# h3poteto/aws-global-accelerator-controller

Hardware: NVIDIA H100
Metric: objects reconciled/sec at 10^6 Service+Ingress; change-set bit-exact vs Go ref (higher is better)
Workload: dtype u8/u32 (bytes and indices)

## Files before the change

### aws-global-accelerator-controller_b200/csrc/gar_common.h

```cpp
#pragma once

#include <stdint.h>
#include <stddef.h>

#include "../../include/garecon.h"

#if defined(__CUDACC__)
#define GAR_HD __host__ __device__ __forceinline__
#define GAR_D __device__ __forceinline__
#else
#define GAR_HD inline
#define GAR_D inline
#endif

#if defined(__CUDA_ARCH__)
#define GAR_ANY(p) __any_sync(0xffffffffu, (p))
#else
bool gar_host_vote(bool p);
#define GAR_ANY(p) gar_host_vote((p))
#endif

typedef uint8_t u8;
typedef uint16_t u16;
typedef uint32_t u32;
// ... 206 lines not shown
#else
  return *p;
#endif
}

GAR_HD Cursor idx_open(const HashIdx &ix, u64 h) {
  u32 b = hash_bucket(h, ix.mask);
  Cursor c;
  c.pos = ix.begin[b];
  c.end = ix.begin[b + 1];
  c.tag = hash_tag(h);
  return c;
}
GAR_HD bool idx_next(const HashIdx &ix, Cursor &c, IdxEntry *out) {
  while (c.pos < c.end) {
    IdxEntry e = load_entry(ix.ent + c.pos++);
    if (e.tag == c.tag) {
      *out = e;
      return true;
    }
  }
  return false;
}
```

### aws-global-accelerator-controller_b200/csrc/gar_pipeline.h

```cpp
#pragma once

#include <stdio.h>
#include <stdlib.h>

#include <initializer_list>

#include "gar_rows.h"

#if defined(__CUDA_ARCH__)
#define GAR_ATOMIC_ADD(p, v) atomicAdd((p), (v))
#else
#define GAR_ATOMIC_ADD(p, v) (*(p) += (v))
#endif


enum Slot {
  S_DERIVED, S_OFLAGS, S_OKEY_HASH, S_STAGE_GA, S_STAGE_R53, S_ANN_R53, S_ANN_NAME, S_ANN_TAGS, S_ANN_LISTEN, S_DPORT_BEGIN, S_DPORTS,
  S_TOK_CODE, S_TOK_NAME, S_TOK_REGION,
  S_ACC_FLAGS, S_ACC_OWNER_KEY, S_ACC_OWNER, S_ACC_THOST, S_ACC_MANAGED, S_ACC_OWNER_HASH, S_ACC_THOST_HASH, S_REC_NAME_HASH, S_VAL_KEY_HASH,
  S_REC_ZONE, S_VAL_REC, S_VAL_CLS, S_VAL_KEY, S_VAL_ORPHAN, S_VAL_LINK, S_ACC_DIGEST,
  S_R53_MODE, S_R53_ACC, S_R53_ACC_DNS, S_PAIR_BEGIN, S_PAIR_OBJ, S_PAIR_HN, S_PAIR_CODE, S_PAIR_ZONE, S_PAIR_REC,
  S_IX_LB, S_IX_OWNER = S_IX_LB + 3, S_IX_THOST = S_IX_OWNER + 3, S_IX_ZONE = S_IX_THOST + 3, S_IX_VAL = S_IX_ZONE + 3,
  S_IX_ALIAS = S_IX_VAL + 3, S_IX_OBJ = S_IX_ALIAS + 3, S_IX_OVN = S_IX_OBJ + 3,
  S_SORT_KEYS = S_IX_OVN + 3, S_SORT_VALS, S_SORT_KEYS_ALT, S_SORT_VALS_ALT, S_SORT_TAGS,
  S_COUNTS, S_STATUS_GA, S_STATUS_R53, S_OPS, S_ERRFLAG, S_IX_EG, S_IX_EG_ENT, S_IX_EG_PAD,
  S_VAL_OBJ, S_ACC_OBJ, S_OBJ_CANON, S_OWN_BEGIN, S_OWN_FILL, S_OWN_ENT, S_OWN_MULTI,
  S_IXA_BEGIN, S_IXA_FILL, S_IXA_ENT, S_IXA_MULTI, S_OVN_FILL, S_OVN_MULTI, S_LB_HASH, S_REC_FLAGS,
  S_NSLOTS
};


struct FClassify {
  DevTables T;
  Work W;
  u32 *derived_public;
  u8 *oflags;
  u32 *errflag;
  GAR_HD void operator()(u32 i) const {
    classify_object(T, W, i);
    W.obj_canon[i] = i;
    u32 dv = W.derived[i];
    if (dv & OBJ_KEY_BAD) GAR_ATOMIC_ADD(errflag, 1u);
    derived_public[i] = dv & 0xFFu;
  }
};
struct FTokenise {
  DevTables T;
  Work W;
  static constexpr int kStageCols = 1;
  static constexpr u32 kStageBytes = 24 * 1024;
// ... 438 lines not shown
  GAR_HD void operator()(u32 k) const { dst[k] = k < 5 ? src[idx[k]] : *extra; }
};
#define GAR_RETRY_WITH_RADIX 1000
#define GAR_REFUSE_EMPTY_CACHE 1001
struct FGatherHeader {
  const u32 *ndports;
  u32 *flags;
  GAR_HD void operator()(u32) const { flags[FW_NDPORTS] = *ndports; }
};
struct FValueJoins {
  DevTables T;
  Work W;
  GAR_HD void operator()(u32 v) const { value_joins(T, W, v); }
};
struct FResolveValue {
  DevTables T;
  Work W;
  GAR_HD void operator()(u32 v) const { resolve_value(T, W, v); }
};
struct FResolveAccel {
  DevTables T;
  Work W;
  GAR_HD void operator()(u32 a) const { resolve_accel(T, W, a); }
};
GAR_HD IdxEntry own_entry(const DevTables &T, const Work &W, u32 x) {
  IdxEntry e;
  e.tag = e.a0 = e.a1 = 0;
  e.s0 = e.s1 = 0;
  if (x < T.a.n_accels) {
    e.row = x;
    return e;
  }
  const u32 v = x - T.a.n_accels, rec = W.val_rec[v];
  const ValLink l = W.val_link[v];
  e.tag = l.alias_row;
  e.row = v;
  e.a0 = rec;
  e.a1 = W.rec_zone[rec] | ((W.rec_flags[rec] & 1) ? VALNAME_HAS_BACKSLASH : 0u);
  e.s0 = l.alias_dns;
  e.s1 = T.a.rec_name[rec];
  return e;
}
GAR_HD u32 own_segment(const DevTables &T, const Work &W, u32 x) {
  const u32 nacc = T.a.n_accels;
  const u32 o = x < nacc ? W.acc_obj[x] : W.val_obj[x - nacc];
  return o == GAR_NONE ? 2 * T.o.n_objects : 2 * o + (x < nacc ? 0u : 1u);
// ... 316 lines not shown
  }

  bool prepared = false;
  u64 n_dports = 0;
  u32 *errflag = nullptr;

  u32 acc_guest_from = 0xFFFFFFFFu;
  u32 sharded = 0;
  bool orphan_sweep = true;
  bool allow_empty_cache = false;

  void alloc_obj_work() {
    const u32 n = T.o.n_objects, nlbi = T.o.n_lbi;
    W.derived = (u32 *)be.ensure(S_DERIVED, 4 * (size_t)(n + 1));
    W.okey_hash = (u64 *)be.ensure(S_OKEY_HASH, 8 * (size_t)(n + 1));
    W.ann_r53 = (gar_str *)be.ensure(S_ANN_R53, 8 * (size_t)(n + 1));
    W.ann_name = (gar_str *)be.ensure(S_ANN_NAME, 8 * (size_t)(n + 1));
    W.ann_tags = (gar_str *)be.ensure(S_ANN_TAGS, 8 * (size_t)(n + 1));
    W.ann_listen = (gar_str *)be.ensure(S_ANN_LISTEN, 8 * (size_t)(n + 1));
    W.dport_begin = (u32 *)be.out_dport_begin(n);
    W.tok_code = (u8 *)be.out_tok_code(nlbi);
    W.tok_name = (gar_str *)be.out_tok_name(nlbi);
    W.tok_region = (gar_str *)be.out_tok_region(nlbi);
    W.r53_mode = (u8 *)be.ensure(S_R53_MODE, (size_t)n + 1);
    W.r53_acc = (u32 *)be.ensure(S_R53_ACC, 4 * (size_t)(n + 1));
    W.r53_acc_dns = (gar_str *)be.ensure(S_R53_ACC_DNS, 8 * (size_t)(n + 1));
    W.obj_canon = (u32 *)be.ensure(S_OBJ_CANON, 4 * (size_t)(n + 1));
  }
  CanonHook canon_hook(u32 b0, u32 b1) const { return CanonHook{W.obj_canon, T.o.slab, b0, b1}; }
  void alloc_work() {
    const u32 nacc = T.a.n_accels, nrec = T.a.n_records, nval = T.a.n_values;
    alloc_obj_work();
    W.acc_flags = (u32 *)be.ensure(S_ACC_FLAGS, 4 * (size_t)(nacc + 1));
    W.acc_owner_key = (gar_str *)be.ensure(S_ACC_OWNER_KEY, 8 * (size_t)(nacc + 1));
    W.acc_owner = (gar_str *)be.ensure(S_ACC_OWNER, 8 * (size_t)(nacc + 1));
    W.acc_thost = (gar_str *)be.ensure(S_ACC_THOST, 8 * (size_t)(nacc + 1));
    W.acc_managed = (gar_str *)be.ensure(S_ACC_MANAGED, 8 * (size_t)(nacc + 1));
    W.acc_owner_hash = (u64 *)be.ensure(S_ACC_OWNER_HASH, 8 * (size_t)(nacc + 1));
    W.acc_thost_hash = (u64 *)be.ensure(S_ACC_THOST_HASH, 8 * (size_t)(nacc + 1));
    W.rec_name_hash = (u64 *)be.ensure(S_REC_NAME_HASH, 8 * (size_t)(nrec + 1));
    W.val_key_hash = (u64 *)be.ensure(S_VAL_KEY_HASH, 8 * (size_t)(nval + 1));
    W.rec_zone = (u32 *)be.ensure(S_REC_ZONE, 4 * (size_t)(nrec + 1));
    W.val_rec = (u32 *)be.ensure(S_VAL_REC, 4 * (size_t)(nval + 1));
    W.val_cls = (u8 *)be.ensure(S_VAL_CLS, nval + 1);
    W.val_key = (gar_str *)be.ensure(S_VAL_KEY, 8 * (size_t)(nval + 1));
    W.val_orphan = (u8 *)be.ensure(S_VAL_ORPHAN, nval + 1);
// ... 82 lines not shown
                      placer(IX_ALIAS, FRowAlias{T, W}), placer(IX_OBJ, FRowObj{T, W}), FIdxMultiList{ixa_begin, ixa_multi});
    const CanonHook canon = P.want[IX_OBJ] ? canon_hook(P.off[IX_OBJ], P.off[IX_OBJ] + P.nb[IX_OBJ]) : CanonHook{};
    be.for_each_dyn("idx_order", ixa_multi, multi_cap, FIdxOrderMulti{ixa_begin, ixa_ent, ixa_multi, overflow, canon});
    if (P.want[IX_LB]) W.ix_lb = group_a_index(IX_LB);
    if (P.want[IX_THOST]) W.ix_thost = group_a_index(IX_THOST);
    if (P.want[IX_ZONE]) W.ix_zone = group_a_index(IX_ZONE);
    if (P.want[IX_ALIAS]) W.ix_alias = group_a_index(IX_ALIAS);
    if (P.want[IX_OBJ]) W.ix_obj = group_a_index(IX_OBJ);
  }
  void resolve_owners(bool link_aliases) {
    const u32 n = T.o.n_objects, nacc = T.a.n_accels, nval = T.a.n_values, nseg = 2 * n;
    u32 *overflow = errflag + FW_IDX_OVERFLOW;
    W.own_begin = (u32 *)be.ensure(S_OWN_BEGIN, 4 * (size_t)(nseg + 2));
    be.fill32(W.own_begin, 0, (size_t)nseg + 1);
    u32 *ovn = nullptr;
    if (!force_radix) {
      ovn_nb = next_pow2(nval / 8 < 16 ? 16 : nval / 8);
      ovn = (u32 *)be.ensure(S_IX_OVN + 0, 4 * (size_t)(ovn_nb + 2));
      be.fill32(ovn, 0, (size_t)ovn_nb + 2);
      W.hist[IX_OVN] = IxHist{ovn, ovn_nb - 1};
    } else {
      W.hist[IX_OVN] = IxHist{nullptr, 0};
    }
    if (link_aliases) be.for_each_multi("value_joins", {nval, nacc}, FValueJoins{T, W}, FResolveAccel{T, W});
    else be.for_each_multi("resolve_owners", {nval, nacc}, FResolveValue{T, W}, FResolveAccel{T, W});
    be.exclusive_scan(W.own_begin, nseg + 1);
    IdxEntry *own = (IdxEntry *)be.ensure(S_OWN_ENT, sizeof(IdxEntry) * ((size_t)nacc + nval + 1));
    if (!force_radix) {
      be.exclusive_scan(ovn, ovn_nb + 1);
      u32 *ovn_cursor = (u32 *)be.ensure(S_OVN_FILL, 4 * (size_t)(ovn_nb + 1));
      IdxEntry *ovn_ent = (IdxEntry *)be.ensure(S_IX_OVN + 1, sizeof(IdxEntry) * (size_t)(nval + 1));
      u32 *ovn_multi = (u32 *)be.ensure(S_OVN_MULTI, 4 * (size_t)(nval / 2 + 3));
      u32 *own_cursor = (u32 *)be.ensure(S_OWN_FILL, 4 * (size_t)(nseg + 1));
      const u32 own_multi_cap = (u32)(((u64)nacc + nval) / 2 + 1);
      u32 *own_multi = (u32 *)be.ensure(S_OWN_MULTI, 4 * (size_t)(own_multi_cap + 2));
      be.copy32(ovn_cursor, ovn, (size_t)ovn_nb + 1);
      be.copy32(own_cursor, W.own_begin, (size_t)nseg + 1);
      be.fill32(ovn_multi, 0, 1);
      be.fill32(own_multi, 0, 1);
      be.for_each_multi("idx_place", {nval, ovn_nb, nacc, nval, nseg}, FIdxPlaceDirect<FRowOvn>{FRowOvn{T, W}, ovn_cursor, ovn_ent, ovn_nb - 1},
                        FIdxMultiList{ovn, ovn_multi}, FOwnPlace{T, W, own_cursor, own, 0}, FOwnPlace{T, W, own_cursor, own, nacc},
                        FIdxMultiList{W.own_begin, own_multi});
      be.for_each_dyn("idx_order", ovn_multi, nval / 2 + 1, FIdxOrderMulti{ovn, ovn_ent, ovn_multi, overflow});
      be.for_each_dyn("idx_order", own_multi, own_multi_cap, FIdxOrderMulti{W.own_begin, own, own_multi, overflow});
      W.ix_ovn = HashIdx{ovn, ovn_ent, ovn_nb - 1};
    } else {
      const u32 nx = nacc + nval;
      u32 *keys = (u32 *)be.ensure(S_SORT_KEYS, 4 * (size_t)(nx + 1));
// ... 27 lines not shown
  }
  void prepare_directory() {
    alloc_work();
    be.fill32(errflag, 0, FW_WORDS);
    arm_group_a((1u << IX_LB) | (1u << IX_THOST));
    if (T.o.n_lbi) be.for_each("tokenise_hostnames", T.o.n_lbi, FTokenise{T, W});
    if (T.a.n_accels) be.for_each("digest_accelerators", T.a.n_accels, FDigestAccel{T, W});
    if (T.a.n_lbs) be.for_each("hash_load_balancers", T.a.n_lbs, FLbHash{T, W});
    finish_group_a();
    u32 fl[FW_WORDS];
    be.download(fl, errflag, sizeof(fl));
    if (fl[FW_IDX_OVERFLOW]) {
      u32 *overflow = errflag + FW_IDX_OVERFLOW;
      W.ix_lb = build_index(S_IX_LB, T.a.n_lbs, 1, FRowLb{T, W}, overflow, true);
      W.ix_thost = build_index(S_IX_THOST, T.a.n_accels, 1, FRowThost{T, W}, overflow, true);
    }
  }

  u32 dport_cap = 0, pair_cap = 0;
  u64 ops_cap = 0;
  bool tiny_caps = false;
  int prepare() {
    const u32 n = T.o.n_objects, nacc = T.a.n_accels, nzone = T.a.n_zones, nrec = T.a.n_records;
    alloc_work();
    if (!force_radix) arm_group_a((1u << IX_LB) | (1u << IX_THOST) | (1u << IX_ZONE) | (1u << IX_ALIAS) | (1u << IX_OBJ));
    stage1();
    listen_ports();

    u32 *overflow = errflag + FW_IDX_OVERFLOW;
    if (!force_radix) {
      finish_group_a();
    } else {
      W.ix_lb = build_index(S_IX_LB, T.a.n_lbs, 1, FRowLb{T, W}, overflow, true);
      W.ix_thost = build_index(S_IX_THOST, nacc, 1, FRowThost{T, W}, overflow, true);
      W.ix_zone = build_index(S_IX_ZONE, nzone, 1, FRowZone{T}, overflow, true);
      W.ix_alias = build_index(S_IX_ALIAS, nrec, 2, FRowAlias{T, W}, overflow, true);
      W.ix_obj = build_index(S_IX_OBJ, n, 1, FRowObj{T, W}, overflow, true, canon_hook(0, 0xFFFFFFFFu));
    }
    resolve_owners(true);
    obj_stale = false;
    owner_indexes = false;
    return GAR_OK;
  }
  void listen_ports() {
    const u32 n = T.o.n_objects;
    be.fill32(W.dport_begin, 0, (size_t)n + 1);
// ... 371 lines not shown
```

### aws-global-accelerator-controller_b200/csrc/gar_rows.h

```cpp
#pragma once

#include "gar_common.h"
#include "gar_json.h"


struct DevTables {
  gar_objects o;
  gar_actual a;
  const u8 *cluster;
  u32 cluster_len;
};

enum {
  OBJ_HAS_NAME_ANN = 1u << 8,
  OBJ_HAS_TAGS_ANN = 1u << 9,
  OBJ_KEY_BAD = 1u << 10,
};

enum {
  ACC_MINE = 1u << 0,
  ACC_OWNER_KEYED = 1u << 1,
  ACC_OWNER_INGRESS = 1u << 2,
  ACC_OWNER_3PART = 1u << 3,
  ACC_HAS_MANAGED = 1u << 4, ACC_HAS_OWNER = 1u << 5, ACC_HAS_THOST = 1u << 6,
// ... 14 lines not shown
  u32 flags;
  u32 lis;
  u32 eg;
  u32 pr_begin;
  u32 ep_begin;
  u16 n_ports, n_eps;
  i32 port0, port1;
  gar_str name;
  gar_str thost;
  gar_str owner_key;
  gar_str ep0;
};
enum {
  ACCD_ENABLED = 1u << 8,
  ACCD_MANAGED_TRUE = 1u << 9,
  ACCD_LIS_NONE = 1u << 10, ACCD_LIS_MANY = 1u << 11,
  ACCD_LIS_UDP = 1u << 12,
  ACCD_EG_NONE = 1u << 13, ACCD_EG_MANY = 1u << 14,
};
struct alignas(16) ValLink {
  u32 alias_row, pad;
  gar_str alias_dns;
};

enum IxId { IX_LB, IX_OWNER, IX_THOST, IX_ZONE, IX_VAL, IX_ALIAS, IX_OBJ, IX_OVN, IX_N };
struct IxHist {
  u32 *cnt;
  u32 mask;
};
#if defined(__CUDA_ARCH__)
#define GAR_HIST_ADD(p) atomicAdd((p), 1u)
#else
#define GAR_HIST_ADD(p) (++*(p))
#endif
GAR_HD void ix_count(const IxHist &h, u64 key_hash) {
  if (h.cnt) GAR_HIST_ADD(&h.cnt[(u32)key_hash & h.mask]);
}

struct Work {
  IxHist hist[IX_N];
  u64 *lb_hash;
  u8 *rec_flags;
  u32 pair_cap;
  u32 dport_cap;
  u32 *derived;
  u64 *okey_hash;
  gar_str *ann_r53;
  gar_str *ann_name;
  gar_str *ann_tags;
  gar_str *ann_listen;
  u32 *dport_begin;
  i32 *dports;
  u8 *tok_code;
  gar_str *tok_name, *tok_region;
  u32 *acc_flags;
  gar_str *acc_owner_key;
  gar_str *acc_owner;
  gar_str *acc_thost;
  gar_str *acc_managed;
  AccDigest *acc_digest;
  u64 *acc_owner_hash;
  u64 *acc_thost_hash;
  u32 *rec_zone;
  u64 *rec_name_hash;
  u32 *val_rec;
  u8 *val_cls;
  gar_str *val_key;
  u64 *val_key_hash;
  u8 *val_orphan;
  ValLink *val_link;
  u32 acc_guest_from;
  u32 sharded;
  u32 *val_obj;
  u32 *acc_obj;
  u32 *obj_canon;
  u32 *own_begin;
  const IdxEntry *own;
// ... 290 lines not shown
  gar_str key = 0;
  const u32 hl = (u32)(sizeof(R53_HERITAGE) - 1);
  u32 fixed = hl + T.cluster_len + 1 + 8 + 1;
  if (s.n >= fixed && HAS_PREFIX_LIT(s, R53_HERITAGE) && streq(substr(s, hl, T.cluster_len), Str{T.cluster, T.cluster_len}) &&
      s.p[hl + T.cluster_len] == ',' && s.p[s.n - 1] == '"') {
    u32 ro = hl + T.cluster_len + 1;
    Str rest = substr(s, ro, s.n - 1 - ro);
    if (HAS_PREFIX_LIT(rest, "service/")) cls = VAL_OWNER_SERVICE;
    else if (HAS_PREFIX_LIT(rest, "ingress/")) cls = VAL_OWNER_INGRESS;
    if (cls) {
      key = GAR_STR(GAR_STR_OFF(ref) + ro + 8, rest.n - 8);
      if (count_slashes(substr(rest, 8, rest.n - 8)) == 1) cls |= VAL_OWNER_3PART;
    }
  }
  W.val_cls[v] = cls;
  W.val_key[v] = key;
  const u64 vkh = cls ? key_hash_kinded((cls & VAL_OWNER_INGRESS) ? 1u : 0u, substr(s, (u32)(GAR_STR_OFF(key) - GAR_STR_OFF(ref)), (u32)GAR_STR_LEN(key))) : 0;
  W.val_key_hash[v] = vkh;
  if (cls) ix_count(W.hist[IX_VAL], vkh);
}
GAR_HD void classify_value(const DevTables &T, const Work &W, u32 v) { classify_value_at(T, W, v, mkstr(T.a.slab, T.a.val_value[v])); }


GAR_HD u32 find_lb(const DevTables &T, const Work &W, Str region, Str name, u32 *state) {
  Cursor c = idx_open(W.ix_lb, key_hash_lb(region, name));
  IdxEntry e;
  while (idx_next(W.ix_lb, c, &e))
    if (streq(mkstr(T.a.slab, e.s0), name) && streq(mkstr(T.a.slab, e.s1), region)) {
      *state = e.a0;
      return e.row;
    }
  return GAR_NONE;
}

struct OwnRange {
  u32 pos, end;
};
GAR_HD OwnRange own_accs(const Work &W, u32 i) {
  const u32 s = 2 * W.obj_canon[i];
  return OwnRange{W.own_begin[s], W.own_begin[s + 1]};
}
GAR_HD OwnRange own_vals(const Work &W, u32 i) {
  const u32 s = 2 * W.obj_canon[i] + 1;
  return OwnRange{W.own_begin[s], W.own_begin[s + 1]};
}

struct OwnerIter {
  Cursor c;
  Str key;
};
GAR_HD OwnerIter owner_open(const Work &W, u64 key_hash, Str key) { return OwnerIter{idx_open(W.ix_owner, key_hash), key}; }
GAR_HD bool owner_match(const DevTables &T, const IdxEntry &e, u32 kind, Str key) {
  return ((((e.a0 & ACC_OWNER_INGRESS) != 0) ? 1u : 0u) == kind) && streq(mkstr(T.a.slab, e.s0), key);
}
GAR_HD u32 owner_next(const DevTables &T, const Work &W, u32 kind, OwnerIter &it) {
  IdxEntry e;
  while (idx_next(W.ix_owner, it.c, &e))
    if (owner_match(T, e, kind, it.key)) return e.row;
  return GAR_NONE;
}

GAR_HD u32 find_by_hostname(const DevTables &T, const Work &W, Str hostname, u32 *first, gar_str *first_dns, u32 *second = nullptr) {
  Cursor c = idx_open(W.ix_thost, key_hash_str(hostname));
  u32 n = 0;
  *first = GAR_NONE;
  if (second) *second = GAR_NONE;
  IdxEntry e;
  while (idx_next(W.ix_thost, c, &e)) {
    if (!streq(mkstr(T.a.slab, e.s0), hostname)) continue;
    if (n == 0) {
      *first = e.row;
      *first_dns = e.s1;
    } else if (second) {
      *second = e.row;
    }
    if (++n >= 2) break;
  }
  return n;
}

GAR_HD bool zone_len_possible(const Work &W, u32 n) {
  u32 b = n < 255 ? n : 255;
  return (W.zone_len_mask[b >> 6] >> (b & 63)) & 1ull;
}
GAR_HD u32 find_hosted_zone(const DevTables &T, const Work &W, Str hostname) {
  Str t = hostname;
  for (;;) {
    if (t.n == 0) return GAR_NONE;
    if (zone_len_possible(W, t.n)) {
      Cursor c = idx_open(W.ix_zone, key_hash_str(t));
      IdxEntry e;
      while (idx_next(W.ix_zone, c, &e)) {
        Str zn = mkstr(T.a.slab, e.s0);
        if (zn.n == t.n + 1 && streq(substr(zn, 0, t.n), t)) return e.row;
      }
    }
    u32 k = find_byte(t, 0, '.');
    if (k >= t.n) return GAR_NONE;
    t = substr(t, k + 1, t.n - k - 1);
  }
}

// ... 6 lines not shown
    }
  if (w == GAR_NONE) return name.n == hostname.n + 1 && name.p[name.n - 1] == '.' && streq(substr(name, 0, hostname.n), hostname);
  if (name.n - 3 != hostname.n + 1) return false;
  if (name.p[name.n - 1] != '.') return false;
  if (w >= hostname.n || hostname.p[w] != '*') return false;
  if (!streq(substr(name, 0, w), substr(hostname, 0, w))) return false;
  u32 tail = hostname.n - w - 1;
  return streq(substr(name, w + 4, tail), substr(hostname, w + 1, tail));
}


GAR_HD Cursor cursor_none() { return Cursor{0, 0, 0}; }
GAR_HD Cursor u_open(const HashIdx &ix, bool active, u64 h) { return active ? idx_open(ix, h) : cursor_none(); }

GAR_HD bool u_bucket_step(const HashIdx &ix, bool searching, Cursor &c, IdxEntry *e) {
  bool step = searching && c.pos < c.end;
  if (step) {
    *e = load_entry(ix.ent + c.pos++);
    return e->tag == c.tag;
  }
  return false;
}
#define U_BUCKET_LOOP(searching_expr, cur) for (; GAR_ANY((searching_expr) && (cur).pos < (cur).end);)

GAR_HD u32 u_find_lb(const DevTables &T, const Work &W, bool active, Str region, Str name, u32 *state) {
  u64 h = hmix(u_hash(active, region), u_hash(active, name));
  Cursor c = u_open(W.ix_lb, active, h);
  u32 found = GAR_NONE;
  U_BUCKET_LOOP(found == GAR_NONE, c) {
    IdxEntry e;
    bool hit = u_bucket_step(W.ix_lb, found == GAR_NONE, c, &e);
    bool eq = u_streq(hit, mkstr(T.a.slab, e.s0), name);
    eq = u_streq(eq, mkstr(T.a.slab, e.s1), region);
    if (eq) {
      found = e.row;
      *state = e.a0;
    }
  }
  return found;
}

GAR_HD u32 u_find_by_hostname(const DevTables &T, const Work &W, bool active, Str hostname, u32 *first, gar_str *first_dns) {
  Cursor c = u_open(W.ix_thost, active, u_hash(active, hostname));
  u32 n = 0;
  *first = GAR_NONE;
  U_BUCKET_LOOP(n < 2, c) {
    IdxEntry e;
    bool hit = u_bucket_step(W.ix_thost, n < 2, c, &e);
    if (u_streq(hit, mkstr(T.a.slab, e.s0), hostname)) {
      if (n == 0) {
        *first = e.row;
        *first_dns = e.s1;
      }
      n++;
    }
  }
  return n;
}

GAR_HD u32 u_find_hosted_zone(const DevTables &T, const Work &W, bool active, Str hostname) {
  Str t = hostname;
  u32 zone = GAR_NONE;
  bool walking = active;
  for (;;) {
    bool round = walking && t.n != 0;
    if (!GAR_ANY(round)) break;
    bool probe = round && zone_len_possible(W, t.n);
    Cursor c = u_open(W.ix_zone, probe, u_hash(probe, t));
    U_BUCKET_LOOP(zone == GAR_NONE, c) {
      IdxEntry e;
      bool hit = u_bucket_step(W.ix_zone, zone == GAR_NONE, c, &e);
      Str zn = mkstr(T.a.slab, e.s0);
      hit = hit && zn.n == t.n + 1;
      if (u_streq(hit, substr(zn, 0, hit ? t.n : 0), t)) zone = e.row;
    }
    u32 k = u_find_byte(round && zone == GAR_NONE, t, 0, '.');
    if (round) {
      if (zone != GAR_NONE || k >= t.n) walking = false;
      else t = substr(t, k + 1, t.n - k - 1);
    }
  }
// ... 151 lines not shown
  u32 fl = W.acc_flags[acc];
  if (!user_managed && !STREQ_LIT(mkstr(A.slab, W.acc_managed[acc]), "true")) return true;
  if (!user_owner) {
    bool ok = (fl & ACC_OWNER_KEYED) && (((fl & ACC_OWNER_INGRESS) ? 1u : 0u) == kind) && streq(mkstr(A.slab, W.acc_owner_key[acc]), object_key(T, i));
    if (!ok) return true;
  }
  if (!user_thost && !streq(mkstr(A.slab, W.acc_thost[acc]), lb_dns)) return true;
  return false;
}

GAR_HD void put_delete_chain(const DevTables &T, OpSink &s, u32 obj, u32 kind, u32 acc) {
  const gar_actual &A = T.a;
  u32 lb = A.acc_lis_begin[acc], le = A.acc_lis_begin[acc + 1];
  u32 lis = GAR_NONE, eg = GAR_NONE;
  if (le - lb == 1) {
    lis = lb;
    u32 eb = A.lis_eg_begin[lis], ee = A.lis_eg_begin[lis + 1];
    if (ee - eb == 1) eg = eb;
  }
  s.put(GAR_OP_HEAD(GAR_OP_GA_DELETE_CHAIN, GAR_CTRL_GA, obj == GAR_NONE ? 0 : kind), obj, 0, acc, lis, eg);
}


GAR_HD bool u_accelerator_changed(const DevTables &T, const Work &W, bool act, u32 i, u32 dv, u32 kind, u32 acc, const AccDigest &d, Str okey, Str lb_dns) {
  const gar_actual &A = T.a;
  bool ch = act && !(d.flags & ACCD_ENABLED);
  bool need = act && !ch;
  Str an = need ? mkstr(A.slab, d.name) : Str{A.slab, 0};
  Str ann = (need && (dv & OBJ_HAS_NAME_ANN)) ? mkstr(T.o.slab, W.ann_name[i]) : Str{T.o.slab, 0};
  bool by_ann = need && ann.n != 0;
  bool eq_ann = u_streq(by_ann, ann, an);
  Str ns = need ? mkstr(T.o.slab, T.o.obj_ns[i]) : Str{T.o.slab, 0};
  Str nm = need ? mkstr(T.o.slab, T.o.obj_name[i]) : Str{T.o.slab, 0};
  bool shape = need && !by_ann && an.n == 9 + ns.n + nm.n &&
               ld64u(an.p) == (kind == GAR_KIND_SERVICE ? 0x2d65636976726573ull  : 0x2d73736572676e69ull ) &&
               an.p[8 + ns.n] == '-';
  bool eq_def = u_streq(shape, substr(an, 8, shape ? ns.n : 0), ns);
  eq_def = u_streq(eq_def, substr(an, 9 + ns.n, eq_def ? nm.n : 0), nm);
  if (need && !(by_ann ? eq_ann : eq_def)) ch = true;
  bool tagcheck = act && !ch;
  bool overlay = tagcheck && (dv & OBJ_HAS_TAGS_ANN);
  if (overlay) ch = accelerator_tags_changed(T, W, i, kind, acc, lb_dns);
  bool sys = tagcheck && !overlay;
  u32 fl = d.flags;
  if (sys && !(fl & ACCD_MANAGED_TRUE)) ch = true;
  bool th = sys && !ch;
  bool th_eq = u_streq(th, th ? mkstr(A.slab, d.thost) : Str{A.slab, 0}, lb_dns);
  if (th && !th_eq) ch = true;
  return ch;
}


GAR_HD void user_tag_effects(const DevTables &T, const Work &W, u32 i, u32 kind, Str okey, bool *keep_visible, bool *user_thost) {
  *keep_visible = true;
  *user_thost = false;
  if (!(W.derived[i] & OBJ_HAS_TAGS_ANN)) return;
  Str tags = mkstr(T.o.slab, W.ann_tags[i]);
  bool m_ok = true, o_ok = true, c_ok = true;
  u32 pos = 0;
  Str piece;
  while (next_piece(tags, &pos, &piece)) {
    TagPiece tp = tag_piece(piece);
    if (!tp.ok) continue;
    if (STREQ_LIT(tp.key, TAG_MANAGED)) m_ok = STREQ_LIT(tp.val, "true");
    else if (STREQ_LIT(tp.key, TAG_OWNER))
      o_ok = tp.val.n == 8 + okey.n && (kind == GAR_KIND_SERVICE ? lit_eq_at(tp.val, 0, "service/") : lit_eq_at(tp.val, 0, "ingress/")) &&
             streq(substr(tp.val, 8, okey.n), okey);
    else if (STREQ_LIT(tp.key, TAG_CLUSTER)) c_ok = streq(tp.val, Str{T.cluster, T.cluster_len});
    else if (STREQ_LIT(tp.key, TAG_THOST)) *user_thost = true;
  }
// ... 22 lines not shown
      kind = o.obj_kind[i];
      if (nj < 1) {
        result = GAR_STATUS(GAR_ST_SKIP_NO_LB, 0, 0);
      } else {
        okey = object_key(T, i);
        if (!(dv & GAR_DV_GA_MANAGED)) {
          const OwnRange ar = own_accs(W, i);
          for (u32 p = ar.pos; p < ar.end; p++) put_delete_chain(T, s, i, kind, W.own[p].row);
          result = GAR_STATUS(GAR_ST_OK, 0, GAR_EV_DELETED);
        } else {
          ensure = true;
        }
      }
    }
  }
  u32 ev = 0;
  bool stop = false;
  u32 prev_lb = GAR_NONE;
  bool pending = false;
  for (u32 j = 0;; j++) {
    bool act = ensure && !stop && j < nj;
    if (!GAR_ANY(act)) break;
    bool probe = false;
    Str hostname{o.slab, 0}, tregion{o.slab, 0}, tname{o.slab, 0};
    if (act) {
      u32 code = W.tok_code[jb + j];
      if (code == GAR_TOK_PANIC) {
        result = GAR_STATUS(GAR_ST_PANIC, 0, ev);
        stop = true;
      } else if (code == GAR_TOK_NOT_AWS) {
      } else if (code >= GAR_TOK_ERR_NOT_ELB) {
        result = GAR_STATUS(GAR_ST_ERR_RETRY, GAR_D_NOT_ELB + (code - GAR_TOK_ERR_NOT_ELB), ev);
        stop = true;
      } else {
        probe = true;
        hostname = mkstr(o.slab, o.lbi_hostname[jb + j]);
        tregion = mkstr(o.slab, W.tok_region[jb + j]);
        tname = mkstr(o.slab, W.tok_name[jb + j]);
      }
    }
    u32 lb_state = 0;
    u32 lb = u_find_lb(T, W, probe, tregion, tname, &lb_state);
    bool have_lb = probe && lb != GAR_NONE;
    Str lb_dns = have_lb ? mkstr(A.slab, A.lb_dns[lb]) : Str{A.slab, 0};
    bool dns_eq = u_streq(have_lb, lb_dns, hostname);
    bool go = false;
    if (probe) {
      if (!have_lb) {
        result = GAR_STATUS(GAR_ST_ERR_RETRY, GAR_D_LB_NOT_FOUND, ev);
        stop = true;
      } else if (!dns_eq) {
        result = GAR_STATUS(GAR_ST_ERR_RETRY, GAR_D_LB_DNS_MISMATCH, ev);
        stop = true;
      } else if (lb_state != GAR_LB_ACTIVE) {
        result = GAR_STATUS(GAR_ST_REQUEUE_30S, 0, ev);
        stop = true;
      } else {
        go = true;
      }
    }
    const bool later = go && prev_lb != GAR_NONE;
    if (later) ga_later_step(T, W, i, kind, okey, jb, j, lb, prev_lb, pending, s, &ev);
    go = go && !later;
    OwnRange oc = go ? own_accs(W, i) : OwnRange{0, 0};
    Str lb_arn = go ? mkstr(A.slab, A.lb_arn[lb]) : Str{A.slab, 0};
    u32 nacc = 0;
    for (;;) {
      bool a = go && !stop && oc.pos < oc.end;
      if (!GAR_ANY(a)) break;
      u32 acc = a ? W.own[oc.pos++].row : GAR_NONE;
      if (a) nacc++;
      AccDigest d;
      d.flags = 0;
      if (a) d = W.acc_digest[acc];
      if (u_accelerator_changed(T, W, a, i, dv, kind, acc, d, okey, lb_dns)) s.put(GAR_OP_HEAD(GAR_OP_GA_UPDATE_ACCEL, GAR_CTRL_GA, kind), i, j, acc, lb, GAR_NONE);
      u32 eg = GAR_NONE;
      if (a) {
        if (d.flags & ACCD_LIS_MANY) {
          result = GAR_STATUS(GAR_ST_ERR_RETRY, GAR_D_TOO_MANY_LISTENERS, ev);
          stop = true;
        } else if (d.flags & ACCD_LIS_NONE) {
          s.put(GAR_OP_HEAD(GAR_OP_GA_CREATE_LISTENER, GAR_CTRL_GA, kind), i, j, acc, GAR_NONE, GAR_NONE);
          s.put(GAR_OP_HEAD(GAR_OP_GA_CREATE_EG, GAR_CTRL_GA, kind), i, j, acc, GAR_NONE, lb);
        } else {
          u32 lis = d.lis;
          bool want_udp = kind == GAR_KIND_SERVICE && (dv & GAR_DV_PROTO_UDP);
          bool changed = ((d.flags & ACCD_LIS_UDP) != 0) != want_udp;
          if (!changed) {
            PortList want = desired_ports(T, W, i);
            if (d.n_ports <= 2 && want.n == d.n_ports && (d.n_ports < 1 || want.p[0] == d.port0) && (d.n_ports < 2 || (want.p[1] == d.port1 && d.port0 != d.port1))) changed = false;
            else changed = ports_changed(PortList{A.pr_from + d.pr_begin, d.n_ports == 0xFFFF ? A.lis_pr_begin[lis + 1] - d.pr_begin : d.n_ports}, want);
          }
          if (changed) s.put(GAR_OP_HEAD(GAR_OP_GA_UPDATE_LISTENER, GAR_CTRL_GA, kind), i, j, acc, lis, GAR_NONE);
          if (d.flags & ACCD_EG_MANY) {
            result = GAR_STATUS(GAR_ST_ERR_RETRY, GAR_D_TOO_MANY_EGS, ev);
            stop = true;
          } else if (d.flags & ACCD_EG_NONE) {
            s.put(GAR_OP_HEAD(GAR_OP_GA_CREATE_EG, GAR_CTRL_GA, kind), i, j, acc, lis, lb);
// ... 28 lines not shown
  bool keep_visible, user_thost;
  user_tag_effects(T, W, i, kind, okey, &keep_visible, &user_thost);
  if (!keep_visible) {
    s.put(GAR_OP_HEAD(GAR_OP_GA_CREATE_CHAIN, GAR_CTRL_GA, kind), i, j, lb, GAR_NONE, GAR_NONE);
    *ev |= GAR_EV_CREATED;
    return;
  }
  Str lb_arn = mkstr(A.slab, A.lb_arn[lb]);
  const bool dns_differs = !user_thost && !streq(mkstr(A.slab, A.lb_dns[lb]), mkstr(A.slab, A.lb_dns[prev_lb]));
  const bool arn_differs = !streq(lb_arn, mkstr(A.slab, A.lb_arn[prev_lb]));
  if (pending) {
    if (dns_differs) s.put(GAR_OP_HEAD(GAR_OP_GA_UPDATE_ACCEL, GAR_CTRL_GA, kind), i, j, GAR_PENDING, lb, GAR_NONE);
    if (arn_differs) s.put(GAR_OP_HEAD(GAR_OP_GA_UPDATE_EG, GAR_CTRL_GA, kind), i, j, GAR_PENDING, GAR_PENDING, lb);
  }
  const OwnRange ar = own_accs(W, i);
  for (u32 p = ar.pos; p < ar.end; p++) {
    const u32 acc = W.own[p].row;
    if (dns_differs) s.put(GAR_OP_HEAD(GAR_OP_GA_UPDATE_ACCEL, GAR_CTRL_GA, kind), i, j, acc, lb, GAR_NONE);
    const AccDigest d = W.acc_digest[acc];
    const bool created = (d.flags & (ACCD_LIS_NONE | ACCD_EG_NONE)) != 0;
    bool replaced = created;
    for (u32 jp = 0; jp < j && !replaced; jp++) {
      if (W.tok_code[jb + jp] > GAR_TOK_NLB) continue;
      u32 st;
      u32 lbp = find_lb(T, W, mkstr(T.o.slab, W.tok_region[jb + jp]), mkstr(T.o.slab, W.tok_name[jb + jp]), &st);
      if (lbp != GAR_NONE && !eg_contains(T, d, mkstr(A.slab, A.lb_arn[lbp]))) replaced = true;
    }
    const bool contains = replaced ? !arn_differs : eg_contains(T, d, lb_arn);
    if (!contains) s.put(GAR_OP_HEAD(GAR_OP_GA_UPDATE_EG, GAR_CTRL_GA, kind), i, j, acc, created ? GAR_PENDING : d.eg, lb);
  }
}


struct OwnedHit {
  u32 v, rec, zone;
  gar_str name;
};
GAR_HD OwnedHit owned_hit(const IdxEntry &e) { return OwnedHit{e.row, e.a0, e.a1 & 0x3FFFFFFFu, e.s1}; }
struct OwnedList {
  const IdxEntry *e;
  u32 n;
};
GAR_HD OwnedList owned_list(const Work &W, u32 i) {
  const OwnRange r = own_vals(W, i);
  return OwnedList{W.own + r.pos, r.end - r.pos};
}
GAR_HD OwnedHit owned_get(const DevTables &, const Work &, const OwnedList &o, u32 k) { return owned_hit(load_entry(o.e + k)); }
constexpr u32 OWNED_CACHE = 8;
struct Owned {
// ... 99 lines not shown
  if (valid) {
    u32 dv = W.derived[i];
    if (dv & GAR_DV_R53_ELIGIBLE) {
      kind = o.obj_kind[i];
      if (!(dv & GAR_DV_R53_ANNOTATED)) {
        r53_cleanup(T, W, i, kind, owned_list(W, i), s);
        result = GAR_STATUS(GAR_ST_OK, 0, GAR_EV_DELETED);
      } else {
        ensure = true;
        hostnames = mkstr(o.slab, W.ann_r53[i]);
        jb = o.obj_lbi_begin[i];
        nj = o.obj_lbi_begin[i + 1] - jb;
      }
    }
  }
  u32 ev = 0;
  bool stop = false;
  bool have_prev = false;
  Str prev_acc_dns{A.slab, 0};
  for (u32 j = 0;; j++) {
    bool act = ensure && !stop && j < nj;
    if (!GAR_ANY(act)) break;
    bool probe = false;
    Str lbhost{o.slab, 0};
    if (act) {
      u32 code = W.tok_code[jb + j];
      if (code == GAR_TOK_PANIC) {
        result = GAR_STATUS(GAR_ST_PANIC, 0, ev);
        stop = true;
      } else if (code == GAR_TOK_NOT_AWS) {
      } else if (code >= GAR_TOK_ERR_NOT_ELB) {
        result = GAR_STATUS(GAR_ST_ERR_RETRY, GAR_D_NOT_ELB + (code - GAR_TOK_ERR_NOT_ELB), ev);
        stop = true;
      } else {
        probe = true;
        lbhost = mkstr(o.slab, o.lbi_hostname[jb + j]);
      }
    }
    u32 acc = GAR_NONE;
    gar_str acc_dns_ref = 0;
    u32 nacc = u_find_by_hostname(T, W, probe, lbhost, &acc, &acc_dns_ref);
    bool go = false;
    if (probe) {
      if (nacc > 1) {
        result = GAR_STATUS(GAR_ST_REQUEUE_60S, GAR_D_ACCEL_MANY, ev);
        stop = true;
      } else if (nacc == 0) {
        result = GAR_STATUS(GAR_ST_REQUEUE_60S, GAR_D_ACCEL_NONE, ev);
        stop = true;
      } else {
        go = true;
      }
    }
    Str acc_dns = go ? mkstr(A.slab, acc_dns_ref) : Str{A.slab, 0};
    if (go) ow = owned_list(W, i);
    bool created = false;
    u32 pos = 0, k = 0;
    for (;;) {
      bool more = go && !stop && pos <= hostnames.n;
      if (!GAR_ANY(more)) break;
      u32 comma = u_find_byte(more, hostnames, pos, ',');
      Str hn = more ? substr(hostnames, pos, comma - pos) : Str{o.slab, 0};
      pos = comma + 1;
      u32 zone = u_find_hosted_zone(T, W, more, hn);
// ... 37 lines not shown
            }
          } else if (!streq(acc_dns, prev_acc_dns)) {
            s.put(GAR_OP_HEAD(GAR_OP_R53_UPSERT_A, GAR_CTRL_R53, kind), i, GAR_R53_SUB(j, k), zone, acc, rec == GAR_NONE ? GAR_PENDING : rec);
          }
        }
        k++;
      }
    }
    if (go && !stop && created) ev |= GAR_EV_CREATED;
    if (go && !stop) {
      have_prev = true;
      prev_acc_dns = acc_dns;
    }
  }
  if (ensure && !stop) result = GAR_STATUS(GAR_ST_OK, 0, ev);
  return result;
}


GAR_HD void r53_prepare(const DevTables &T, const Work &W, u32 i, u32 t, bool valid, u32 *status) {
  const gar_objects &o = T.o;
  u32 mode = R53_MODE_DONE, st = GAR_STATUS(GAR_ST_IGNORED, 0, 0), npairs = 0;
  bool probe = false;
  Str lbhost{o.slab, 0}, hostnames{o.slab, 0};
  if (valid) {
    u32 dv = W.derived[i];
    if (dv & GAR_DV_R53_ELIGIBLE) {
      u32 jb = o.obj_lbi_begin[i], nj = o.obj_lbi_begin[i + 1] - jb;
      if (!(dv & GAR_DV_R53_ANNOTATED) || nj > 1) {
        mode = R53_MODE_OBJECT;
      } else if (nj == 0) {
        st = GAR_STATUS(GAR_ST_OK, 0, 0);
      } else {
        u32 code = W.tok_code[jb];
        if (code == GAR_TOK_PANIC) st = GAR_STATUS(GAR_ST_PANIC, 0, 0);
        else if (code == GAR_TOK_NOT_AWS) st = GAR_STATUS(GAR_ST_OK, 0, 0);
        else if (code >= GAR_TOK_ERR_NOT_ELB) st = GAR_STATUS(GAR_ST_ERR_RETRY, GAR_D_NOT_ELB + (code - GAR_TOK_ERR_NOT_ELB), 0);
        else {
          probe = true;
          lbhost = mkstr(o.slab, o.lbi_hostname[jb]);
          hostnames = mkstr(o.slab, W.ann_r53[i]);
        }
      }
    }
  }
  u32 acc = GAR_NONE;
  gar_str acc_dns = 0;
  u32 nacc = u_find_by_hostname(T, W, probe, lbhost, &acc, &acc_dns);
  bool go = false;
  if (probe) {
    if (nacc > 1) st = GAR_STATUS(GAR_ST_REQUEUE_60S, GAR_D_ACCEL_MANY, 0);
    else if (nacc == 0) st = GAR_STATUS(GAR_ST_REQUEUE_60S, GAR_D_ACCEL_NONE, 0);
    else go = true;
  }
  u32 pos = 0;
  for (;;) {
    bool more = go && pos <= hostnames.n;
    if (!GAR_ANY(more)) break;
    u32 comma = u_find_byte(more, hostnames, pos, ',');
    if (more) {
      npairs++;
      pos = comma + 1;
    }
  }
  if (go) mode = R53_MODE_PAIRS;
  if (valid) {
    W.r53_mode[i] = (u8)mode;
    W.r53_acc[i] = acc;
    W.r53_acc_dns[i] = acc_dns;
    W.pair_begin[t] = npairs;
    if (mode == R53_MODE_DONE) status[t] = st;
// ... 424 lines not shown
```

Measured before the change: 186.9 million.

## Precompute per-LB-ingress lookups in a dedicated pass and reuse in reconcilers

Adds a per-load-balancer-ingress pass (run alongside existing resolve kernels) that looks up the LB and accelerator-by-hostname once and stores verdicts, ARNs, DNS refs and counts in a compact LbiRes table. The GA, R53 and EG-replacement paths then read this table instead of repeating warp-uniform hash lookups and string comparisons, and the accelerator hostname check can skip a string compare when the cached accelerator matches. The lookup pass uses a prefetching cursor that issues the first bucket entry load for both indexes before walking them. The cost is an extra buffer and pass over all ingresses, including ones whose objects never reach these lookups, plus a new row-count limit check.

After: 193.6 million (median of 6 runs). +3.6%, better.

```diff
diff --git a/aws-global-accelerator-controller_b200/csrc/gar_common.h b/aws-global-accelerator-controller_b200/csrc/gar_common.h
--- a/aws-global-accelerator-controller_b200/csrc/gar_common.h
+++ b/aws-global-accelerator-controller_b200/csrc/gar_common.h
@@ -252,3 +252,27 @@
   }
   return false;
 }
+struct PreCursor {
+  Cursor c;
+  IdxEntry e;
+  bool loaded;
+};
+GAR_HD PreCursor idx_open_pre(const HashIdx &ix, u64 h) {
+  PreCursor p;
+  p.c = idx_open(ix, h);
+  p.loaded = p.c.pos < p.c.end;
+  if (p.loaded) p.e = load_entry(ix.ent + p.c.pos);
+  return p;
+}
+GAR_HD bool idx_next(const HashIdx &ix, PreCursor &p, IdxEntry *out) {
+  while (p.c.pos < p.c.end) {
+    if (!p.loaded) p.e = load_entry(ix.ent + p.c.pos);
+    p.loaded = false;
+    p.c.pos++;
+    if (p.e.tag == p.c.tag) {
+      *out = p.e;
+      return true;
+    }
+  }
+  return false;
+}
diff --git a/aws-global-accelerator-controller_b200/csrc/gar_pipeline.h b/aws-global-accelerator-controller_b200/csrc/gar_pipeline.h
--- a/aws-global-accelerator-controller_b200/csrc/gar_pipeline.h
+++ b/aws-global-accelerator-controller_b200/csrc/gar_pipeline.h
@@ -25,7 +25,7 @@
   S_SORT_KEYS = S_IX_OVN + 3, S_SORT_VALS, S_SORT_KEYS_ALT, S_SORT_VALS_ALT, S_SORT_TAGS,
   S_COUNTS, S_STATUS_GA, S_STATUS_R53, S_OPS, S_ERRFLAG, S_IX_EG, S_IX_EG_ENT, S_IX_EG_PAD,
   S_VAL_OBJ, S_ACC_OBJ, S_OBJ_CANON, S_OWN_BEGIN, S_OWN_FILL, S_OWN_ENT, S_OWN_MULTI,
-  S_IXA_BEGIN, S_IXA_FILL, S_IXA_ENT, S_IXA_MULTI, S_OVN_FILL, S_OVN_MULTI, S_LB_HASH, S_REC_FLAGS,
+  S_IXA_BEGIN, S_IXA_FILL, S_IXA_ENT, S_IXA_MULTI, S_OVN_FILL, S_OVN_MULTI, S_LB_HASH, S_REC_FLAGS, S_LBI_RES,
   S_NSLOTS
 };
 
@@ -510,6 +510,11 @@
   DevTables T;
   Work W;
   GAR_HD void operator()(u32 a) const { resolve_accel(T, W, a); }
+};
+struct FLbiResolve {
+  DevTables T;
+  Work W;
+  GAR_HD void operator()(u32 r) const { lbi_resolve(T, W, r); }
 };
 GAR_HD IdxEntry own_entry(const DevTables &T, const Work &W, u32 x) {
   IdxEntry e;
@@ -872,6 +877,7 @@
     W.tok_code = (u8 *)be.out_tok_code(nlbi);
     W.tok_name = (gar_str *)be.out_tok_name(nlbi);
     W.tok_region = (gar_str *)be.out_tok_region(nlbi);
+    W.lbi_res = (LbiRes *)be.ensure(S_LBI_RES, sizeof(LbiRes) * (size_t)(nlbi + 1));
     W.r53_mode = (u8 *)be.ensure(S_R53_MODE, (size_t)n + 1);
     W.r53_acc = (u32 *)be.ensure(S_R53_ACC, 4 * (size_t)(n + 1));
     W.r53_acc_dns = (gar_str *)be.ensure(S_R53_ACC_DNS, 8 * (size_t)(n + 1));
@@ -1000,8 +1006,9 @@
     } else {
       W.hist[IX_OVN] = IxHist{nullptr, 0};
     }
-    if (link_aliases) be.for_each_multi("value_joins", {nval, nacc}, FValueJoins{T, W}, FResolveAccel{T, W});
-    else be.for_each_multi("resolve_owners", {nval, nacc}, FResolveValue{T, W}, FResolveAccel{T, W});
+    const u32 nlbi = T.o.n_lbi;
+    if (link_aliases) be.for_each_multi("value_joins", {nval, nacc, nlbi}, FValueJoins{T, W}, FResolveAccel{T, W}, FLbiResolve{T, W});
+    else be.for_each_multi("resolve_owners", {nval, nacc, nlbi}, FResolveValue{T, W}, FResolveAccel{T, W}, FLbiResolve{T, W});
     be.exclusive_scan(W.own_begin, nseg + 1);
     IdxEntry *own = (IdxEntry *)be.ensure(S_OWN_ENT, sizeof(IdxEntry) * ((size_t)nacc + nval + 1));
     if (!force_radix) {
@@ -1075,6 +1082,7 @@
   bool tiny_caps = false;
   int prepare() {
     const u32 n = T.o.n_objects, nacc = T.a.n_accels, nzone = T.a.n_zones, nrec = T.a.n_records;
+    if (T.a.n_lbs > LBI_ROW_MASK || nacc > LBI_ROW_MASK) return GAR_E_INVALID;
     alloc_work();
     if (!force_radix) arm_group_a((1u << IX_LB) | (1u << IX_THOST) | (1u << IX_ZONE) | (1u << IX_ALIAS) | (1u << IX_OBJ));
     stage1();
diff --git a/aws-global-accelerator-controller_b200/csrc/gar_rows.h b/aws-global-accelerator-controller_b200/csrc/gar_rows.h
--- a/aws-global-accelerator-controller_b200/csrc/gar_rows.h
+++ b/aws-global-accelerator-controller_b200/csrc/gar_rows.h
@@ -60,6 +60,19 @@
   u32 alias_row, pad;
   gar_str alias_dns;
 };
+struct alignas(32) LbiRes {
+  u32 lb;
+  u32 acc;
+  gar_str acc_dns;
+  gar_str lb_dns;
+  gar_str lb_arn;
+};
+enum { LBI_OK = 0, LBI_DNS_MISMATCH = 1, LBI_NOT_ACTIVE = 2, LBI_NOT_FOUND = 3 };
+#define LBI_ROW_MASK 0x3FFFFFFFu
+GAR_HD u32 lbi_verdict(const LbiRes &r) { return r.lb >> 30; }
+GAR_HD u32 lbi_lb(const LbiRes &r) { return r.lb == GAR_NONE ? GAR_NONE : r.lb & LBI_ROW_MASK; }
+GAR_HD u32 lbi_acc_count(const LbiRes &r) { return r.acc >> 30; }
+GAR_HD u32 lbi_acc(const LbiRes &r) { return lbi_acc_count(r) ? r.acc & LBI_ROW_MASK : GAR_NONE; }
 
 enum IxId { IX_LB, IX_OWNER, IX_THOST, IX_ZONE, IX_VAL, IX_ALIAS, IX_OBJ, IX_OVN, IX_N };
 struct IxHist {
@@ -91,6 +104,7 @@
   i32 *dports;
   u8 *tok_code;
   gar_str *tok_name, *tok_region;
+  LbiRes *lbi_res;
   u32 *acc_flags;
   gar_str *acc_owner_key;
   gar_str *acc_owner;
@@ -427,8 +441,8 @@
 GAR_HD void classify_value(const DevTables &T, const Work &W, u32 v) { classify_value_at(T, W, v, mkstr(T.a.slab, T.a.val_value[v])); }
 
 
-GAR_HD u32 find_lb(const DevTables &T, const Work &W, Str region, Str name, u32 *state) {
-  Cursor c = idx_open(W.ix_lb, key_hash_lb(region, name));
+template <class C>
+GAR_HD u32 lb_walk(const DevTables &T, const Work &W, C &c, Str region, Str name, u32 *state) {
   IdxEntry e;
   while (idx_next(W.ix_lb, c, &e))
     if (streq(mkstr(T.a.slab, e.s0), name) && streq(mkstr(T.a.slab, e.s1), region)) {
@@ -437,6 +451,10 @@
     }
   return GAR_NONE;
 }
+GAR_HD u32 find_lb(const DevTables &T, const Work &W, Str region, Str name, u32 *state) {
+  Cursor c = idx_open(W.ix_lb, key_hash_lb(region, name));
+  return lb_walk(T, W, c, region, name, state);
+}
 
 struct OwnRange {
   u32 pos, end;
@@ -465,8 +483,8 @@
   return GAR_NONE;
 }
 
-GAR_HD u32 find_by_hostname(const DevTables &T, const Work &W, Str hostname, u32 *first, gar_str *first_dns, u32 *second = nullptr) {
-  Cursor c = idx_open(W.ix_thost, key_hash_str(hostname));
+template <class C>
+GAR_HD u32 thost_walk(const DevTables &T, const Work &W, C &c, Str hostname, u32 *first, gar_str *first_dns, u32 *second = nullptr) {
   u32 n = 0;
   *first = GAR_NONE;
   if (second) *second = GAR_NONE;
@@ -483,6 +501,33 @@
   }
   return n;
 }
+GAR_HD u32 find_by_hostname(const DevTables &T, const Work &W, Str hostname, u32 *first, gar_str *first_dns, u32 *second = nullptr) {
+  Cursor c = idx_open(W.ix_thost, key_hash_str(hostname));
+  return thost_walk(T, W, c, hostname, first, first_dns, second);
+}
+
+GAR_HD void lbi_resolve(const DevTables &T, const Work &W, u32 r) {
+  if (W.tok_code[r] > GAR_TOK_NLB) return;
+  const gar_actual &A = T.a;
+  const Str host = mkstr(T.o.slab, T.o.lbi_hostname[r]);
+  const Str region = mkstr(T.o.slab, W.tok_region[r]), name = mkstr(T.o.slab, W.tok_name[r]);
+  PreCursor cl = idx_open_pre(W.ix_lb, key_hash_lb(region, name)), ch = idx_open_pre(W.ix_thost, key_hash_str(host));
+  LbiRes res;
+  u32 state = 0;
+  const u32 lb = lb_walk(T, W, cl, region, name, &state);
+  res.lb_dns = lb != GAR_NONE ? A.lb_dns[lb] : 0;
+  res.lb_arn = lb != GAR_NONE ? A.lb_arn[lb] : 0;
+  u32 acc = GAR_NONE;
+  res.acc_dns = 0;
+  const u32 nacc = thost_walk(T, W, ch, host, &acc, &res.acc_dns);
+  res.acc = (nacc << 30) | (acc & LBI_ROW_MASK);
+  res.lb = GAR_NONE;
+  if (lb != GAR_NONE) {
+    const u32 v = !streq(mkstr(A.slab, res.lb_dns), host) ? LBI_DNS_MISMATCH : state != GAR_LB_ACTIVE ? LBI_NOT_ACTIVE : LBI_OK;
+    res.lb = (v << 30) | lb;
+  }
+  W.lbi_res[r] = res;
+}
 
 GAR_HD bool zone_len_possible(const Work &W, u32 n) {
   u32 b = n < 255 ? n : 255;
@@ -535,41 +580,6 @@
   return false;
 }
 #define U_BUCKET_LOOP(searching_expr, cur) for (; GAR_ANY((searching_expr) && (cur).pos < (cur).end);)
-
-GAR_HD u32 u_find_lb(const DevTables &T, const Work &W, bool active, Str region, Str name, u32 *state) {
-  u64 h = hmix(u_hash(active, region), u_hash(active, name));
-  Cursor c = u_open(W.ix_lb, active, h);
-  u32 found = GAR_NONE;
-  U_BUCKET_LOOP(found == GAR_NONE, c) {
-    IdxEntry e;
-    bool hit = u_bucket_step(W.ix_lb, found == GAR_NONE, c, &e);
-    bool eq = u_streq(hit, mkstr(T.a.slab, e.s0), name);
-    eq = u_streq(eq, mkstr(T.a.slab, e.s1), region);
-    if (eq) {
-      found = e.row;
-      *state = e.a0;
-    }
-  }
-  return found;
-}
-
-GAR_HD u32 u_find_by_hostname(const DevTables &T, const Work &W, bool active, Str hostname, u32 *first, gar_str *first_dns) {
-  Cursor c = u_open(W.ix_thost, active, u_hash(active, hostname));
-  u32 n = 0;
-  *first = GAR_NONE;
-  U_BUCKET_LOOP(n < 2, c) {
-    IdxEntry e;
-    bool hit = u_bucket_step(W.ix_thost, n < 2, c, &e);
-    if (u_streq(hit, mkstr(T.a.slab, e.s0), hostname)) {
-      if (n == 0) {
-        *first = e.row;
-        *first_dns = e.s1;
-      }
-      n++;
-    }
-  }
-  return n;
-}
 
 GAR_HD u32 u_find_hosted_zone(const DevTables &T, const Work &W, bool active, Str hostname) {
   Str t = hostname;
@@ -767,7 +777,8 @@
 }
 
 
-GAR_HD bool u_accelerator_changed(const DevTables &T, const Work &W, bool act, u32 i, u32 dv, u32 kind, u32 acc, const AccDigest &d, Str okey, Str lb_dns) {
+GAR_HD bool u_accelerator_changed(const DevTables &T, const Work &W, bool act, u32 i, u32 dv, u32 kind, u32 acc, const AccDigest &d, Str okey, Str lb_dns,
+                                  bool thost_eq) {
   const gar_actual &A = T.a;
   bool ch = act && !(d.flags & ACCD_ENABLED);
   bool need = act && !ch;
@@ -790,7 +801,8 @@
   u32 fl = d.flags;
   if (sys && !(fl & ACCD_MANAGED_TRUE)) ch = true;
   bool th = sys && !ch;
-  bool th_eq = u_streq(th, th ? mkstr(A.slab, d.thost) : Str{A.slab, 0}, lb_dns);
+  bool th_cmp = th && !thost_eq;
+  bool th_eq = u_streq(th_cmp, th_cmp ? mkstr(A.slab, d.thost) : Str{A.slab, 0}, lb_dns) || (th && thost_eq);
   if (th && !th_eq) ch = true;
   return ch;
 }
@@ -859,7 +871,6 @@
     bool act = ensure && !stop && j < nj;
     if (!GAR_ANY(act)) break;
     bool probe = false;
-    Str hostname{o.slab, 0}, tregion{o.slab, 0}, tname{o.slab, 0};
     if (act) {
       u32 code = W.tok_code[jb + j];
       if (code == GAR_TOK_PANIC) {
@@ -871,36 +882,35 @@
         stop = true;
       } else {
         probe = true;
-        hostname = mkstr(o.slab, o.lbi_hostname[jb + j]);
-        tregion = mkstr(o.slab, W.tok_region[jb + j]);
-        tname = mkstr(o.slab, W.tok_name[jb + j]);
-      }
-    }
-    u32 lb_state = 0;
-    u32 lb = u_find_lb(T, W, probe, tregion, tname, &lb_state);
-    bool have_lb = probe && lb != GAR_NONE;
-    Str lb_dns = have_lb ? mkstr(A.slab, A.lb_dns[lb]) : Str{A.slab, 0};
-    bool dns_eq = u_streq(have_lb, lb_dns, hostname);
+      }
+    }
+    LbiRes res;
+    res.lb = GAR_NONE;
+    res.lb_dns = res.lb_arn = 0;
+    if (probe) res = W.lbi_res[jb + j];
+    const u32 lb = lbi_lb(res);
     bool go = false;
     if (probe) {
-      if (!have_lb) {
+      const u32 v = lbi_verdict(res);
+      if (v == LBI_NOT_FOUND) {
         result = GAR_STATUS(GAR_ST_ERR_RETRY, GAR_D_LB_NOT_FOUND, ev);
         stop = true;
-      } else if (!dns_eq) {
+      } else if (v == LBI_DNS_MISMATCH) {
         result = GAR_STATUS(GAR_ST_ERR_RETRY, GAR_D_LB_DNS_MISMATCH, ev);
         stop = true;
-      } else if (lb_state != GAR_LB_ACTIVE) {
+      } else if (v == LBI_NOT_ACTIVE) {
         result = GAR_STATUS(GAR_ST_REQUEUE_30S, 0, ev);
         stop = true;
       } else {
         go = true;
       }
     }
+    const Str lb_dns = mkstr(A.slab, res.lb_dns);
     const bool later = go && prev_lb != GAR_NONE;
     if (later) ga_later_step(T, W, i, kind, okey, jb, j, lb, prev_lb, pending, s, &ev);
     go = go && !later;
     OwnRange oc = go ? own_accs(W, i) : OwnRange{0, 0};
-    Str lb_arn = go ? mkstr(A.slab, A.lb_arn[lb]) : Str{A.slab, 0};
+    Str lb_arn = go ? mkstr(A.slab, res.lb_arn) : Str{A.slab, 0};
     u32 nacc = 0;
     for (;;) {
       bool a = go && !stop && oc.pos < oc.end;
@@ -910,7 +920,8 @@
       AccDigest d;
       d.flags = 0;
       if (a) d = W.acc_digest[acc];
-      if (u_accelerator_changed(T, W, a, i, dv, kind, acc, d, okey, lb_dns)) s.put(GAR_OP_HEAD(GAR_OP_GA_UPDATE_ACCEL, GAR_CTRL_GA, kind), i, j, acc, lb, GAR_NONE);
+      const bool thost_eq = a && acc == lbi_acc(res);
+      if (u_accelerator_changed(T, W, a, i, dv, kind, acc, d, okey, lb_dns, thost_eq)) s.put(GAR_OP_HEAD(GAR_OP_GA_UPDATE_ACCEL, GAR_CTRL_GA, kind), i, j, acc, lb, GAR_NONE);
       u32 eg = GAR_NONE;
       if (a) {
         if (d.flags & ACCD_LIS_MANY) {
@@ -985,9 +996,8 @@
     bool replaced = created;
     for (u32 jp = 0; jp < j && !replaced; jp++) {
       if (W.tok_code[jb + jp] > GAR_TOK_NLB) continue;
-      u32 st;
-      u32 lbp = find_lb(T, W, mkstr(T.o.slab, W.tok_region[jb + jp]), mkstr(T.o.slab, W.tok_name[jb + jp]), &st);
-      if (lbp != GAR_NONE && !eg_contains(T, d, mkstr(A.slab, A.lb_arn[lbp]))) replaced = true;
+      const LbiRes rp = W.lbi_res[jb + jp];
+      if (lbi_lb(rp) != GAR_NONE && !eg_contains(T, d, mkstr(A.slab, rp.lb_arn))) replaced = true;
     }
     const bool contains = replaced ? !arn_differs : eg_contains(T, d, lb_arn);
     if (!contains) s.put(GAR_OP_HEAD(GAR_OP_GA_UPDATE_EG, GAR_CTRL_GA, kind), i, j, acc, created ? GAR_PENDING : d.eg, lb);
@@ -1133,7 +1143,6 @@
     bool act = ensure && !stop && j < nj;
     if (!GAR_ANY(act)) break;
     bool probe = false;
-    Str lbhost{o.slab, 0};
     if (act) {
       u32 code = W.tok_code[jb + j];
       if (code == GAR_TOK_PANIC) {
@@ -1145,12 +1154,16 @@
         stop = true;
       } else {
         probe = true;
-        lbhost = mkstr(o.slab, o.lbi_hostname[jb + j]);
-      }
-    }
-    u32 acc = GAR_NONE;
+      }
+    }
+    u32 acc = GAR_NONE, nacc = 0;
     gar_str acc_dns_ref = 0;
-    u32 nacc = u_find_by_hostname(T, W, probe, lbhost, &acc, &acc_dns_ref);
+    if (probe) {
+      const LbiRes res = W.lbi_res[jb + j];
+      nacc = lbi_acc_count(res);
+      acc = lbi_acc(res);
+      acc_dns_ref = res.acc_dns;
+    }
     bool go = false;
     if (probe) {
       if (nacc > 1) {
@@ -1234,7 +1247,8 @@
   const gar_objects &o = T.o;
   u32 mode = R53_MODE_DONE, st = GAR_STATUS(GAR_ST_IGNORED, 0, 0), npairs = 0;
   bool probe = false;
-  Str lbhost{o.slab, 0}, hostnames{o.slab, 0};
+  u32 lbi = 0;
+  Str hostnames{o.slab, 0};
   if (valid) {
     u32 dv = W.derived[i];
     if (dv & GAR_DV_R53_ELIGIBLE) {
@@ -1250,15 +1264,20 @@
         else if (code >= GAR_TOK_ERR_NOT_ELB) st = GAR_STATUS(GAR_ST_ERR_RETRY, GAR_D_NOT_ELB + (code - GAR_TOK_ERR_NOT_ELB), 0);
         else {
           probe = true;
-          lbhost = mkstr(o.slab, o.lbi_hostname[jb]);
+          lbi = jb;
           hostnames = mkstr(o.slab, W.ann_r53[i]);
         }
       }
     }
   }
-  u32 acc = GAR_NONE;
+  u32 acc = GAR_NONE, nacc = 0;
   gar_str acc_dns = 0;
-  u32 nacc = u_find_by_hostname(T, W, probe, lbhost, &acc, &acc_dns);
+  if (probe) {
+    const LbiRes res = W.lbi_res[lbi];
+    nacc = lbi_acc_count(res);
+    acc = lbi_acc(res);
+    acc_dns = res.acc_dns;
+  }
   bool go = false;
   if (probe) {
     if (nacc > 1) st = GAR_STATUS(GAR_ST_REQUEUE_60S, GAR_D_ACCEL_MANY, 0);
```
